# XiandaGuo/OpenStereo

Measured on AMD Instinct MI355X. Metric: stereo-pairs/s at 540x960 D=192 (GwcNet fwd), higher is better.
Workload: dtype f32 via f16x3 split-MFMA (hi/lo fp16 operands, f32 accumulate; HBM tensors f32); 1 GPU; GwcNet-gc inference, SceneFlow-shaped 540x960 padded to 544x960, D=192, G=40 + 12ch concat (BASELINE configs[1]); weights=deterministic synthetic (sharpened), random-init architecture, sub_batch_streams=3, parallelism=independent pairs x1, precision=f16x3, launch=hipGraph replay

## Files before the change

### include/openstereo_amd.h

```cpp
#ifndef OPENSTEREO_AMD_H
#define OPENSTEREO_AMD_H

#include <stddef.h>

#ifdef __cplusplus
extern "C" {
#endif

#define OSA_ABI_VERSION 8
#define OSA_META_FLOATS 128

enum { OSA_NCDHW = 0, OSA_NDHWC = 1 };
enum { OSA_ACT_NONE = 0, OSA_ACT_RELU = 1, OSA_ACT_LEAKY = 2, OSA_ACT_RELU6 = 3, OSA_ACT_SIGMOID = 4, OSA_ACT_TANH = 5 };
enum { OSA_GATE_RAW = 16 };
#define OSA_GATE_CHANNELS(n) ((int)((unsigned)(n) << 16))
enum { OSA_IN_SPLIT = 32, OSA_OUT_SPLIT = 64, OSA_RES_SPLIT = 128, OSA_REDIR_SPLIT = 256 };
enum { OSA_RES_AFTER_ACT = 512 };

int         osa_abi_version(void);
const char* osa_last_error(void);
const char* osa_target_arch(void);

int osa_build_volume_f32(const float* left_gwc, const float* right_gwc, int C, int num_groups,
                         const float* left_cat, const float* right_cat, int Cc,
// ... 310 lines not shown
                     float* out, float* workspace, size_t workspace_bytes, void* stream);
int osa_channel_sums_multi(const void* const* dys, int n_items, int dy_f16, int dy_cs, long long P, int C,
                           float* out, float* workspace, size_t workspace_bytes, void* stream);
int osa_channel_affine(const void* u, int u_f16, int u_cs, const void* v, int v_f16, int v_cs,
                       const float* a, const float* b, const float* c0, void* out, int out_cs,
                       long long P, int C, int relu, void* stream);

size_t osa_instnorm_workspace_floats(int B, long long HW, int C);
int osa_instnorm_nhwc_f32(const float* x, float* y, int B, long long HW, int C, int xCs, int yCs, float eps, int act, float slope,
                          float* workspace, float* y_meta, void* stream);

long long osa_conv3d_march_launches(void);

long long osa_conv3d_march_s2_launches(void);

int osa_conv_b_ring_mask(int mask);
long long osa_conv_b_ring_launches(void);

int osa_volume_walk_step(int step);
long long osa_volume_walk_launches(void);

int osa_build_volume_nhwc_split_eligible(const float* left_cat, const float* right_cat, const float* vol, int C, int num_groups,
                                         int gwc_stride, int Cc, int cat_stride, int vol_channels, int c_off, int W, int maxdisp);
int osa_build_volume_nhwc_split_f16x3(const float* left_gwc, const float* right_gwc, int C, int num_groups, int gwc_stride,
                                      const float* left_cat, const float* right_cat, int Cc, int cat_stride,
                                      float* vol, int vol_channels, int c_off,
                                      int B, int H, int W, int maxdisp, int mask_left_concat,
                                      const float* gwc_meta, const float* cat_meta, float* vol_meta, void* stream);

#ifdef __cplusplus
// ... 4 lines not shown
```

### openstereo_amd/_lib.py

```python
from __future__ import annotations

import ctypes as C
import os
import threading

_HERE = os.path.dirname(os.path.abspath(__file__))
LIB_PATH = os.environ.get("OSA_LIB_PATH") or os.path.join(_HERE, "lib", "libopenstereo_amd.so")

_lock = threading.Lock()
_lib = None

c_fp = C.c_void_p
c_i = C.c_int
c_f = C.c_float
c_st = C.c_void_p
c_ll = C.c_longlong


class F16x3Ranges(C.Structure):
    _fields_ = [("x_meta", C.c_void_p), ("residual_meta", C.c_void_p), ("redir_meta", C.c_void_p),
                ("y_meta", C.c_void_p), ("bound_coef", C.c_void_p), ("redir_bound_coef", C.c_void_p), ("weight_scale", C.c_void_p)]


c_rng = C.POINTER(F16x3Ranges)
# ... 152 lines not shown
                                     c_i, c_f, c_st]),
    "osa_deconv2d_nhwc_f16": (c_i, [c_fp, c_fp, c_fp, c_fp, c_fp, c_fp,
                                    c_i, c_i, c_i, c_i, c_i,
                                    c_i, c_i, c_i,
                                    c_i, c_i, c_i,
                                    c_fp, c_i, c_i, c_f, c_st]),
    "osa_instnorm_workspace_floats": (C.c_size_t, [c_i, c_ll, c_i]),
    "osa_instnorm_nhwc_f32": (c_i, [c_fp, c_fp, c_i, c_ll, c_i, c_i, c_i, c_f, c_i, c_f, c_fp, c_fp, c_st]),
    "osa_conv3d_wgrad_ws_multi": (c_i, [c_i, c_fp, c_fp, c_i, c_fp] + [c_i] * 22 + [c_fp, c_fp, c_i, c_i, c_fp, C.c_size_t, c_st]),
    "osa_channel_sums_workspace_bytes": (C.c_size_t, [c_ll, c_i]),
    "osa_channel_affine": (c_i, [c_fp, c_i, c_i, c_fp, c_i, c_i, c_fp, c_fp, c_fp, c_fp, c_i, c_ll, c_i, c_i, c_st]),
    "osa_channel_sums_multi": (c_i, [c_fp, c_i, c_i, c_i, c_ll, c_i, c_fp, c_fp, C.c_size_t, c_st]),
    "osa_channel_sums": (c_i, [c_fp, c_i, c_i, c_fp, c_i, c_i, c_fp, c_fp, c_fp, c_i, c_ll, c_i, c_fp, c_fp, C.c_size_t, c_st]),
    "osa_conv3d_march_launches": (c_ll, []),
    "osa_conv3d_march_s2_launches": (c_ll, []),
    "osa_conv_b_ring_mask": (c_i, [c_i]),
    "osa_conv_b_ring_launches": (c_ll, []),
    "osa_volume_walk_step": (c_i, [c_i]),
    "osa_volume_walk_launches": (c_ll, []),
    "osa_build_volume_nhwc_split_eligible": (c_i, [c_fp, c_fp, c_fp, c_i, c_i, c_i, c_i, c_i, c_i, c_i, c_i, c_i]),
    "osa_build_volume_nhwc_split_f16x3": (c_i, [c_fp, c_fp, c_i, c_i, c_i, c_fp, c_fp, c_i, c_i, c_fp, c_i, c_i,
                                                c_i, c_i, c_i, c_i, c_i, c_fp, c_fp, c_fp, c_st]),
    "osa_softargmin_f32": (c_i, [c_fp, c_fp, c_i, c_i, c_i, c_i, c_st]),
    "osa_softmax_softargmin_f32": (c_i, [c_fp, c_fp, c_fp, c_i, c_i, c_i, c_i, c_st]),
    "osa_upsample_softargmin_f32": (c_i, [c_fp, c_fp, c_i, c_i, c_i, c_i, c_i, c_i, c_i, c_i, c_st]),
    "osa_softargmin_var_f32": (c_i, [c_fp, c_fp, c_fp, c_fp, c_i, c_i, c_i, c_i, c_st]),
    "osa_softmax_softargmin_var_f32": (c_i, [c_fp, c_fp, c_fp, c_i, c_i, c_i, c_i, c_st]),
    "osa_upsample_softargmin_var_f32": (c_i, [c_fp, c_fp, c_fp, c_i, c_i, c_i, c_i, c_i, c_i, c_i, c_i, c_st]),
    "osa_softargmin_var_bwd_f32": (c_i, [c_fp, c_fp, c_fp, c_fp, c_fp, c_fp, c_i, c_i, c_i, c_i, c_st]),
    "osa_softmax_softargmin_var_bwd_f32": (c_i, [c_fp, c_fp, c_fp, c_fp, c_i, c_i, c_i, c_i, c_st]),
# ... 13 lines not shown
        if _lib is not None:
            return _lib
        if not os.path.exists(LIB_PATH):
            raise EngineError(
                f"{LIB_PATH} is missing: build it with `python -m openstereo_amd.build` "
                "(hipcc, gfx950). There is no CPU fallback.")
        lib = C.CDLL(LIB_PATH)
        for name, (res, args) in SIGNATURES.items():
            fn = getattr(lib, name)
            fn.restype = res
            fn.argtypes = args
        if lib.osa_abi_version() != abi_version(lib):
            raise EngineError(f"ABI version mismatch: library reports {lib.osa_abi_version()}, include/openstereo_amd.h declares {abi_version(lib)}")
        if os.environ.get("OSA_B_RING_MASK"):
            lib.osa_conv_b_ring_mask(int(os.environ["OSA_B_RING_MASK"], 0))
        if os.environ.get("OSA_VOL_WALK"):
            lib.osa_volume_walk_step(int(os.environ["OSA_VOL_WALK"]))
        _lib = lib
    return _lib


_abi = None


def abi_version(lib=None) -> int:
    global _abi
    if _abi is None:
        import re
        hdr = os.path.join(os.path.dirname(os.path.abspath(__file__)), "..", "include", "openstereo_amd.h")
        try:
# ... 22 lines not shown
```

### openstereo_amd/build.py

```python
from __future__ import annotations

import os
import shutil
import subprocess
import sys
from concurrent.futures import ThreadPoolExecutor

HERE = os.path.dirname(os.path.abspath(__file__))
CSRC = os.path.join(HERE, "csrc")
LIBDIR = os.path.join(HERE, "lib")
OBJDIR = os.path.join(LIBDIR, "obj")
LIBNAME = "libopenstereo_amd.so"
SOURCES = ["api.hip", "volume.hip", "conv3d.hip", "conv_inst_f32.hip", "conv_inst_f16x3.hip", "conv_inst_f16.hip", "conv_march.hip", "softargmin.hip", "layout.hip", "refine.hip", "backward.hip", "wgrad.hip", "geometry.hip", "dwconv.hip", "norm.hip", "gru_train.hip"]
ARCH = "gfx950"
HIPCC_FLAGS = ["-O3", "-std=c++17", f"--offload-arch={ARCH}", "-fPIC", "-ffp-contract=off",
               "-Wall", "-Wno-unused-function"]
NO_PACKED_F32 = ["-Xclang", "-target-feature", "-Xclang", "-packed-fp32-ops"]
HIPCC_FLAGS += NO_PACKED_F32
EXTRA_FLAGS: dict = {}


def _hipcc() -> str:
    exe = shutil.which("hipcc") or "/opt/rocm/bin/hipcc"
    if not os.path.exists(exe):
# ... 3 lines not shown

def _stale(target: str, deps: list[str]) -> bool:
    if not os.path.exists(target):
        return True
    t = os.path.getmtime(target)
    return any(os.path.getmtime(d) > t for d in deps)


def lib_path() -> str:
    return os.path.join(LIBDIR, LIBNAME)


def build(force: bool = False, verbose: bool = True) -> str:
    os.makedirs(OBJDIR, exist_ok=True)
    hipcc = _hipcc()
    headers = [os.path.join(CSRC, "osa_common.h"), os.path.join(CSRC, "conv_kernel.h"), os.path.join(CSRC, "conv_march.h"), os.path.join(CSRC, "conv_inst.h"), os.path.join(CSRC, "conv_inst_impl.h"), os.path.join(CSRC, "conv_cfgs.def"),
               os.path.join(HERE, "..", "include", "openstereo_amd.h")]

    def compile_one(src: str) -> str:
        s = os.path.join(CSRC, src)
        o = os.path.join(OBJDIR, src.replace(".hip", ".o"))
        if force or _stale(o, [s, os.path.abspath(__file__)] + headers):
            cmd = [hipcc, *HIPCC_FLAGS, *EXTRA_FLAGS.get(src, []), "-c", s, "-o", o]
            if verbose:
                print("[build]", " ".join(cmd), flush=True)
            subprocess.check_call(cmd)
        return o

    with ThreadPoolExecutor(max_workers=min(len(SOURCES), os.cpu_count() or 1)) as ex:
        objs = list(ex.map(compile_one, SOURCES))
    out = lib_path()
# ... 13 lines not shown
```

### openstereo_amd/csrc/conv3d.hip

```cpp
#include "conv_kernel.h"
#include "conv_inst.h"

namespace osa {

struct KernelCfg {
    const char* name;
    int M, N;
    int TD, TH, TW, threads;
    int ks;
    int table, idx;
};

static const KernelCfg g_cfgs[] = {
#define OSA_CFG_X(RING, MT, NT, WM, WN, TH, TW)                                                                  \
    { #MT "x" #NT "_" #WM "x" #WN "_" #TH "x" #TW, WM * MT * 32, WN * NT * 32, WM * MT * 32 / (TH * TW), TH, TW, WM * WN * 64, 0, 0, -1 },
#define OSA_KS_X(MT, NT, WM, WN, TH, TW, KS)
#include "conv_cfgs.def"
#undef OSA_CFG_X
#undef OSA_KS_X
};
constexpr int N_CFGS = sizeof(g_cfgs) / sizeof(g_cfgs[0]);

static const KernelCfg g_ks_cfgs[] = {
#define OSA_CFG_X(RING, MT, NT, WM, WN, TH, TW)
// ... 148 lines not shown
    const double mfma_per_wave = (double)a.nchunks * a.T * ((double)k.M * k.N / 1024.0 / waves) * (prec == PREC_F16X3 ? 3.0 : 8.0);
    const double tap_us = mfma_per_wave * (prec == PREC_F16X3 ? 32.0 : 64.0) / 2000.0;
    const double bytes = (double)a.LD * a.LH * a.LW * 64.0 * a.nchunks + (double)k.M * (deconv ? 8 : 1) * k.N * 4.0 * (a.res || a.rx ? 2 : 1);
    const double mem_us = bytes / (4.0e6 / 256.0);
    double step_us = tap_us > mem_us ? tap_us : mem_us;
    if ((tap_us + mem_us) / slots > step_us) step_us = (tap_us + mem_us) / slots;
    { const int o = exp_int("OSA_STAG_PCT", 100); step_us *= o / 100.0; }
    { const int o = exp_int("OSA_STAG_US10", 0); if (o) step_us = o / 10.0; }
    a.stag_ticks = (int)(step_us * 100.0 + 0.5);
    a.stag_n = slots * 256; a.stag_cus = 256;
    if (exp_int("OSA_STAG_PRINT", 0)) fprintf(stderr, "[stagger] %s slots %d tap %.2f us mem %.2f us step %.2f us\n", k.name, slots, tap_us, mem_us, step_us);
}

int launch_conv_march(ConvArgs& a, hipStream_t st, const char* what);
int launch_conv_march_s2(ConvArgs& a, hipStream_t st, const char* what);
void wgrad_set_multi_tile(int on);
void march_s2_set_waves(int w);

static int g_b_ring_mask = (1 << 1) | (1 << 2) | (1 << 3) | (1 << 4) | (1 << 13) | (1 << 29) | (1 << 27);
static long long g_b_ring_launches = 0;
static int g_b_ring_mask_value() { return g_b_ring_mask; }

static int launch_conv(ConvArgs& a, int stride, int prec, hipStream_t st, const char* what,
                       const KernelCfg* forced = nullptr) {
#ifdef OSA_EXPERIMENTS
    if (!forced) {
        const int r = launch_conv_pipe(a, stride, prec, st, what);
        if (r != 0) return r < 0 ? r : 0;
    }
#endif
// ... 662 lines not shown
    for (int t = 0; t < d.T; ++t) { a.td[t] = d.dz[t]; a.th[t] = d.dy[t]; a.tw[t] = d.dx[t]; }
    for (int c = 0; c < 8; ++c) a.cls_end[c] = d.cls_end[c];
    a.nchunks = nchunks_of(Ci); a.CoP = pad32(Co);
    a.act = act; a.slope = slope; a.oscale = oscale;
    if (prec == PREC_F16 && f16_units(a, flat ? "deconv2d" : "deconv3d")) return -1;
    if (rx) {
        OSA_REQUIRE(!flat && !residual && !gate_logits, "deconv3d_redir: residual / gate cannot be combined with the fused redir branch");
        OSA_REQUIRE(rw_packed && rCi > 0 && rCi <= 64 && rCi % 4 == 0 && rxCs >= rCi && rxCs % 4 == 0 && ((size_t)rx & 15) == 0,
                    "deconv3d_redir: redir input needs <= 64 channels (multiple of 4), stride >= channels, 16-byte alignment (Ci=%d stride=%d)", rCi, rxCs);
        OSA_REQUIRE((long long)a.Do * a.Ho * a.Wo * rxCs < (1ll << 31), "deconv3d_redir: redir input too large");
        a.rx = rx; a.rxCs = rxCs; a.rCi = rCi; a.rw = reinterpret_cast<const float4*>(rw_packed);
        a.rscale = rscale; a.rshift = rshift; a.roscale = roscale;
    }
    set_ranges(a, rng);
    if (check_split_ranges(a, prec, flat ? "deconv2d" : "deconv3d")) return -1;
    return launch_conv(a, 1, prec, (hipStream_t)stream, flat ? "deconv2d" : "deconv3d",
                       flat ? &g_deconv_flat_cfg : (rx ? (rCi > 32 ? &g_deconv_redir64_cfg : &g_deconv_redir_cfg) : &g_deconv_cfg));
}

#define OSA_DECONV_PARAMS                                                                       \
    const float* x, const float* w_packed, const float* scale, const float* shift,             \
    const float* residual, float* y, int B, int Di, int Hi, int Wi, int Ci, int xCs,           \
    int Co, int yCs, int rCs, int k, int pad, int opad, const float* gate_logits, int gCs, int act, float slope
#define OSA_DECONV_ARGS                                                                         \
    x, w_packed, scale, shift, residual, y, B, Di, Hi, Wi, Ci, xCs, Co, yCs, rCs, k, pad, opad, \
    gate_logits, gCs, act, slope

extern "C" int osa_deconv3d_ndhwc_f32(OSA_DECONV_PARAMS, void* stream) {
    return deconv3d_impl(OSA_DECONV_ARGS, PREC_F32, 1.f, stream);
}
// ... 184 lines not shown
```

### openstereo_amd/csrc/conv_kernel.h

```cpp
#pragma once
#include "osa_common.h"
#include <cstdlib>
#include <cstring>

#include <type_traits>

namespace osa {

typedef float f32x16 __attribute__((ext_vector_type(16)));
typedef _Float16 f16x8 __attribute__((ext_vector_type(8)));
typedef unsigned int u32x4 __attribute__((ext_vector_type(4)));

enum { PREC_F32 = 0, PREC_F16X3 = 1, PREC_F16 = 2 };

constexpr int CC = 16;
constexpr int VS = CC + 4;
constexpr int JO = CC / 8;
constexpr int MAX_TAPS = 64;

struct ConvArgs {
    const float* x; const float4* w; const float* scale; const float* shift; const float* res; float* y;
    const float* gate; int gCs;
    int B, Di, Hi, Wi, Ci, xCs;
    int Do, Ho, Wo, Co, yCs, rCs;
// ... 171 lines not shown
            else if (lane_in) row[lane] = zero;
        } else if (lane_in) row[lane] = zero;
    }
}

__device__ __forceinline__ void wait_vmcnt(const int n) {
    switch (n) {
        case 0: asm volatile("s_waitcnt vmcnt(0)" ::: "memory"); break;
        case 1: asm volatile("s_waitcnt vmcnt(1)" ::: "memory"); break;
        case 2: asm volatile("s_waitcnt vmcnt(2)" ::: "memory"); break;
        case 3: asm volatile("s_waitcnt vmcnt(3)" ::: "memory"); break;
        case 4: asm volatile("s_waitcnt vmcnt(4)" ::: "memory"); break;
        case 5: asm volatile("s_waitcnt vmcnt(5)" ::: "memory"); break;
        default: asm volatile("s_waitcnt vmcnt(6)" ::: "memory"); break;
    }
}

#ifdef OSA_TRACE_ON
constexpr int TRACE_SLOTS = 32, TRACE_WAVES = 4, TRACE_EVENTS = 40;
static __device__ unsigned long long g_trace[TRACE_SLOTS * TRACE_WAVES * TRACE_EVENTS];
#define OSA_TRACE(ev) do { if ((p.dbg & 256) && (tid & 63) == 0 && blockIdx.y == 0 && blockIdx.x % 97 == 0 && blockIdx.x / 97 < TRACE_SLOTS && (tid >> 6) < TRACE_WAVES && (ev) < TRACE_EVENTS) \
    g_trace[((blockIdx.x / 97) * TRACE_WAVES + (tid >> 6)) * TRACE_EVENTS + (ev)] = wall_clock64(); } while (0)
#else
#define OSA_TRACE(ev) do {} while (0)
#endif

template <int PREC, int NCLS, int TU, int MT, int NT, int WM, int WN, int TH, int TW, int REDIR = 0, int OUTS = 0, int PIPE = 0, int KS = 1, int BL = 0>
#ifndef OSA_S2_U
#define OSA_S2_U 12
#endif
// ... 1077 lines not shown
```

### openstereo_amd/csrc/conv_march.h

```cpp
#pragma once
#include "conv_kernel.h"

namespace osa {

template <int NWV, int TW>
struct MarchGeo {
    static constexpr int MT = 2;
    static constexpr int RPT = 32 / TW;
    static constexpr int TH = NWV * MT * RPT;
    static constexpr int LH = TH + 2, LW = TW + 2;
    static constexpr int VQ = 5;
    static constexpr int ROWQ = (TW == 16) ? ((LW * VQ + 15) / 16 * 16) : LW * VQ;
    static constexpr int NPI = (LH * ROWQ + 63) / 64;
    static constexpr int PLANEQ = NPI * 64;
    static constexpr int NP = (NPI + NWV - 1) / NWV;
    static constexpr int NTHR = NWV * 64;
    static constexpr int BRING = 4;
    static constexpr int BSTEPQ = 6 * 64;
    static constexpr size_t lds_bytes() { return (size_t)2 * PLANEQ * 16 + (size_t)BRING * BSTEPQ * 16; }
    static_assert((size_t)NWV * 32 * 36 * 4 <= (size_t)PLANEQ * 16, "epilogue tiles must fit into one plane buffer");
    static_assert(NP <= 7, "one piece per wave and step, all of them forced home by the waits of steps 2..8");
};

__device__ const float4 g_march_zeros[4] = {};

template <int NWV, int TW, int OUTS, int INS>
__global__ __launch_bounds__(NWV * 64, 2) void conv_march_kernel(const ConvArgs p, const int dseg, const int nseg) {
    using G = MarchGeo<NWV, TW>;
    constexpr int MT = G::MT, TH = G::TH, ROWQ = G::ROWQ, VQ = G::VQ, PLANEQ = G::PLANEQ, NTHR = G::NTHR, NP = G::NP, NPI = G::NPI;
    extern __shared__ __attribute__((aligned(16))) float4 smem[];
    float4* const bring = smem + 2 * PLANEQ;

    const int tid = threadIdx.x, lane = tid & 63;
    const int wm = __builtin_amdgcn_readfirstlane(tid >> 6);
    const int col = lane & 31, hh = lane >> 5;

    unsigned bid = xcd_remap(blockIdx.x, gridDim.x);
    const int twi = bid % p.tilesW; bid /= p.tilesW;
    const int thi = bid % p.tilesH; bid /= p.tilesH;
    const int seg = bid % nseg;
// ... 32 lines not shown
            for (int r = 0; r < 16; ++r) acc[s][m][r] = 0.f;

    const int bstep = 2 * p.CoP;
    const int tstep = 2 * bstep;
    const int nch = p.nchunks;

    const int cq = (lane & 7) * 4, vsub = lane >> 3;
    const int c8 = (lane & 3) * 8, vs2 = lane >> 2;
    const int actk = p.act & 15;
    const float act_ns = (actk == OSA_ACT_NONE) ? 1.f : ((actk == OSA_ACT_LEAKY) ? p.slope : 0.f);
    const bool act_relu = actk == OSA_ACT_RELU;
    const size_t ovox_b = (size_t)b * p.Do * p.Ho * p.Wo;
    float* const yb = p.y + ovox_b * p.yCs;
    const float* const resb = p.res ? p.res + ovox_b * p.rCs : nullptr;

    auto dma = [&](const char* src, const unsigned lds_byte) {
        const unsigned m0v = __builtin_amdgcn_readfirstlane(lds_byte);
        unsigned keep;
        asm volatile("s_mov_b32 %0, m0\n\ts_mov_b32 m0, %2\n\ts_nop 0\n\tglobal_load_lds_dwordx4 %1, off\n\ts_mov_b32 m0, %0"
                     : "=&s"(keep) : "v"(src), "s"(m0v) : "memory");
    };
    const unsigned smem_lds = (unsigned)(size_t)(__attribute__((address_space(3))) char*)smem;
    const unsigned bring_lds = smem_lds + 2u * PLANEQ * 16u;
    const char* const zsrc = reinterpret_cast<const char*>(g_march_zeros);

    constexpr int PERW = 384 / NWV, NI = (PERW + 63) / 64;
    unsigned boff[NI];
#pragma unroll
    for (int i = 0; i < NI; ++i) {
        const int j = wm * PERW + i * 64 + lane, f = (j >> 6) < 6 ? (j >> 6) : 5;
        boff[i] = (unsigned)(((f >> 1) * 9 * tstep + (f & 1) * bstep + (j & 63)) * 16);
    }
    auto dma_b = [&](const int slot, const int ch, const int khw) {
        const char* base = reinterpret_cast<const char*>(p.w) + (size_t)(ch * 27 + khw) * tstep * 16;
#pragma unroll
        for (int i = 0; i < NI; ++i)
            if ((i + 1) * 64 <= PERW || i * 64 + lane < PERW)
                dma(base + boff[i], bring_lds + (unsigned)((slot * 384 + wm * PERW + i * 64) * 16));
    };
// ... 202 lines not shown
```

### openstereo_amd/csrc/conv_march.hip

```cpp
#include "conv_march.h"
#include "conv_march_s2.h"

namespace osa {

static long long g_march_launches = 0;
long long march_launches() { return g_march_launches; }

struct MarchCfg { int nwv, tw, th; size_t lds; void (*fn[2][2])(const ConvArgs, int, int); };
#define OSA_MARCH_CFG(NWV, TW) { NWV, TW, MarchGeo<NWV, TW>::TH, MarchGeo<NWV, TW>::lds_bytes(),                      \
                                 { { conv_march_kernel<NWV, TW, 0, 0>, conv_march_kernel<NWV, TW, 0, 1> },            \
                                   { conv_march_kernel<NWV, TW, 1, 0>, conv_march_kernel<NWV, TW, 1, 1> } } }
static const MarchCfg g_march_cfgs[] = {
    OSA_MARCH_CFG(4, 16),
    OSA_MARCH_CFG(4, 32),
};

int launch_conv_march(ConvArgs& a, hipStream_t st, const char* what) {
    if (!exp_int("OSA_MARCH", 1)) return 0;
    if (a.T != 27 || a.Co != 32 || a.CoP != 32 || a.Di < 3 || a.gate || a.rx) return 0;
    if (a.Ci % 16 != 0) return 0;
    const int actk = a.act & 15;
    if (actk > OSA_ACT_LEAKY || (a.act & (OSA_GATE_RAW | OSA_RES_AFTER_ACT)) || ((unsigned)a.act >> 16)) return 0;
    if ((a.yCs & 3) || ((size_t)a.y & 15) || (a.res && ((a.rCs & 3) || ((size_t)a.res & 15)))) return 0;
    if ((long long)a.Do * a.Ho * a.Wo * (a.yCs > a.rCs ? a.yCs : a.rCs) >= (1ll << 31)) return 0;
// ... 91 lines not shown

int launch_conv_march_s2(ConvArgs& a, hipStream_t st, const char* what) {
    if (a.T != 27 || a.Co != 64 || a.CoP != 64 || a.Di < 2 || a.gate || a.rx || a.res) return 0;
    if (a.Ci % 16 != 0 || a.xCs % 16 != 0) return 0;
    if (!(a.act & OSA_IN_SPLIT) || !(a.act & OSA_OUT_SPLIT)) return 0;
    const int actk = a.act & 15;
    if (actk > OSA_ACT_LEAKY || (a.act & (OSA_GATE_RAW | OSA_RES_AFTER_ACT)) || ((unsigned)a.act >> 16)) return 0;
    if ((a.yCs % 16) || ((size_t)a.y & 15) || ((size_t)a.x & 15)) return 0;
    if ((long long)a.Do * a.Ho * a.Wo * a.yCs >= (1ll << 31)) return 0;
    if ((long long)a.Hi * a.Wi * a.xCs >= (1ll << 29)) return 0;
    const int r = g_march_s2_waves == 8 ? launch_conv_march_s2_t<8>(a, st, what) : launch_conv_march_s2_t<4>(a, st, what);
    if (r == 1) ++g_march_s2_launches;
    return r;
}

}

extern "C" long long osa_conv3d_march_launches(void) { return osa::march_launches(); }
extern "C" long long osa_conv3d_march_s2_launches(void) { return osa::march_s2_launches(); }
```

### openstereo_amd/csrc/conv_march_s2.h

```cpp
#pragma once
#include "conv_kernel.h"

namespace osa {

template <int NWV_>
struct MarchS2Geo {
    static constexpr int NWV = NWV_, TW = 32, TH = NWV_ / 2;
    static constexpr int LH = 2 * TH + 1, LW = 2 * TW + 1, NEV = TW + 1;
    static constexpr int NVOX = LH * LW;
    static constexpr int NPI = (NVOX * 4 + 63) / 64;
    static constexpr int PLANEQ = NPI * 64;
    static constexpr int NP = (NPI + NWV - 1) / NWV;
    static constexpr int BRING = 3, BSTEPQ = 12 * 64;
    static constexpr int NIB = NWV == 8 ? 2 : 3;
    static constexpr size_t lds_bytes() { return (size_t)2 * PLANEQ * 16 + (size_t)BRING * BSTEPQ * 16; }
    static_assert((size_t)NWV * 32 * 36 * 4 <= (size_t)PLANEQ * 16, "epilogue tiles must fit into one plane buffer");
};

__device__ const float4 g_march_s2_zeros[4] = {};

template <int N>
__device__ __forceinline__ void wait_vmcnt_c() {
    static_assert(N >= 0 && N <= 15, "vmcnt immediate");
    if constexpr (N == 0) asm volatile("s_waitcnt vmcnt(0)" ::: "memory");
    else if constexpr (N == 1) asm volatile("s_waitcnt vmcnt(1)" ::: "memory");
    else if constexpr (N == 2) asm volatile("s_waitcnt vmcnt(2)" ::: "memory");
    else if constexpr (N == 3) asm volatile("s_waitcnt vmcnt(3)" ::: "memory");
    else if constexpr (N == 4) asm volatile("s_waitcnt vmcnt(4)" ::: "memory");
    else if constexpr (N == 5) asm volatile("s_waitcnt vmcnt(5)" ::: "memory");
    else if constexpr (N == 6) asm volatile("s_waitcnt vmcnt(6)" ::: "memory");
    else if constexpr (N == 7) asm volatile("s_waitcnt vmcnt(7)" ::: "memory");
    else if constexpr (N == 8) asm volatile("s_waitcnt vmcnt(8)" ::: "memory");
    else asm volatile("s_waitcnt vmcnt(9)" ::: "memory");
}
// ... 28 lines not shown
    unsigned amax_seen = 0u;
    if (p.out_meta) amax_seen = amax_peek(p.out_meta);

    f32x16 acc0, acc1;
#pragma unroll
    for (int r = 0; r < 16; ++r) { acc0[r] = 0.f; acc1[r] = 0.f; }

    const int CoP = p.CoP;
    const int nch = p.nchunks;
    const int c8 = (lane & 3) * 8, vs2 = lane >> 2;
    const int actk = p.act & 15;
    const float act_ns = (actk == OSA_ACT_NONE) ? 1.f : ((actk == OSA_ACT_LEAKY) ? p.slope : 0.f);
    const bool act_relu = actk == OSA_ACT_RELU;
    float* const yb = p.y + (size_t)b * p.Do * p.Ho * p.Wo * p.yCs;

    auto dma = [&](const char* src, const unsigned lds_byte) {
        const unsigned m0v = __builtin_amdgcn_readfirstlane(lds_byte);
        unsigned keep;
        asm volatile("s_mov_b32 %0, m0\n\ts_mov_b32 m0, %2\n\ts_nop 0\n\tglobal_load_lds_dwordx4 %1, off\n\ts_mov_b32 m0, %0"
                     : "=&s"(keep) : "v"(src), "s"(m0v) : "memory");
    };
    const unsigned smem_lds = (unsigned)(size_t)(__attribute__((address_space(3))) char*)smem;
    const unsigned bring_lds = smem_lds + 2u * PLANEQ * 16u;
    const char* const zsrc = reinterpret_cast<const char*>(g_march_s2_zeros);

    unsigned boff[NIB], bdst[NIB];
#pragma unroll
    for (int i = 0; i < NIB; ++i) {
        const int f = NWV == 8 ? (i == 0 ? wv : 8 + (wv & 3)) : wv * 3 + i;
        const int kw = f >> 2, hl = (f >> 1) & 1, n = f & 1;
        boff[i] = (unsigned)((kw * 4 * CoP + hl * 2 * CoP + hh * CoP + n * 32 + col) * 16);
        bdst[i] = (unsigned)(f * 64 * 16);
    }
    auto dma_b = [&](const int slot, const int ch, const int kh, const int kd) {
        const char* base = reinterpret_cast<const char*>(p.w) + (size_t)((ch * 27 + kd * 9 + kh * 3) * 4 * CoP) * 16;
#pragma unroll
        for (int i = 0; i < NIB; ++i) dma(base + boff[i], bring_lds + (unsigned)(slot * G::BSTEPQ * 16) + bdst[i]);
    };

// ... 154 lines not shown
```

Measured before the change: 196.6 stereo-pairs/s.

## Add plane-walking transposed-conv3d kernel with fused redir 1x1 epilogue

Measured after the change: 200.2 stereo-pairs/s (median of 6 runs). +1.8%, better.

```diff
diff --git a/include/openstereo_amd.h b/include/openstereo_amd.h
--- a/include/openstereo_amd.h
+++ b/include/openstereo_amd.h
@@ -7,7 +7,7 @@
 extern "C" {
 #endif
 
-#define OSA_ABI_VERSION 8
+#define OSA_ABI_VERSION 9
 #define OSA_META_FLOATS 128
 
 enum { OSA_NCDHW = 0, OSA_NDHWC = 1 };
@@ -348,6 +348,10 @@
 
 long long osa_conv3d_march_s2_launches(void);
 
+int osa_deconv_walk(int enable);
+int osa_deconv_walk_segment_planes(int planes);
+long long osa_deconv3d_walk_launches(void);
+
 int osa_conv_b_ring_mask(int mask);
 long long osa_conv_b_ring_launches(void);
 
diff --git a/openstereo_amd/_lib.py b/openstereo_amd/_lib.py
--- a/openstereo_amd/_lib.py
+++ b/openstereo_amd/_lib.py
@@ -190,6 +190,9 @@
     "osa_channel_sums": (c_i, [c_fp, c_i, c_i, c_fp, c_i, c_i, c_fp, c_fp, c_fp, c_i, c_ll, c_i, c_fp, c_fp, C.c_size_t, c_st]),
     "osa_conv3d_march_launches": (c_ll, []),
     "osa_conv3d_march_s2_launches": (c_ll, []),
+    "osa_deconv_walk": (c_i, [c_i]),
+    "osa_deconv_walk_segment_planes": (c_i, [c_i]),
+    "osa_deconv3d_walk_launches": (c_ll, []),
     "osa_conv_b_ring_mask": (c_i, [c_i]),
     "osa_conv_b_ring_launches": (c_ll, []),
     "osa_volume_walk_step": (c_i, [c_i]),
@@ -233,6 +236,8 @@
             raise EngineError(f"ABI version mismatch: library reports {lib.osa_abi_version()}, include/openstereo_amd.h declares {abi_version(lib)}")
         if os.environ.get("OSA_B_RING_MASK"):
             lib.osa_conv_b_ring_mask(int(os.environ["OSA_B_RING_MASK"], 0))
+        if os.environ.get("OSA_DECONV_WALK"):
+            lib.osa_deconv_walk(int(os.environ["OSA_DECONV_WALK"], 0))
         if os.environ.get("OSA_VOL_WALK"):
             lib.osa_volume_walk_step(int(os.environ["OSA_VOL_WALK"]))
         _lib = lib
diff --git a/openstereo_amd/build.py b/openstereo_amd/build.py
--- a/openstereo_amd/build.py
+++ b/openstereo_amd/build.py
@@ -41,7 +41,7 @@
 def build(force: bool = False, verbose: bool = True) -> str:
     os.makedirs(OBJDIR, exist_ok=True)
     hipcc = _hipcc()
-    headers = [os.path.join(CSRC, "osa_common.h"), os.path.join(CSRC, "conv_kernel.h"), os.path.join(CSRC, "conv_march.h"), os.path.join(CSRC, "conv_inst.h"), os.path.join(CSRC, "conv_inst_impl.h"), os.path.join(CSRC, "conv_cfgs.def"),
+    headers = [os.path.join(CSRC, "osa_common.h"), os.path.join(CSRC, "conv_kernel.h"), os.path.join(CSRC, "conv_march.h"), os.path.join(CSRC, "conv_march_s2.h"), os.path.join(CSRC, "conv_deconv_walk.h"), os.path.join(CSRC, "conv_inst.h"), os.path.join(CSRC, "conv_inst_impl.h"), os.path.join(CSRC, "conv_cfgs.def"),
                os.path.join(HERE, "..", "include", "openstereo_amd.h")]
 
     def compile_one(src: str) -> str:
diff --git a/openstereo_amd/csrc/conv3d.hip b/openstereo_amd/csrc/conv3d.hip
--- a/openstereo_amd/csrc/conv3d.hip
+++ b/openstereo_amd/csrc/conv3d.hip
@@ -186,6 +186,7 @@
 
 int launch_conv_march(ConvArgs& a, hipStream_t st, const char* what);
 int launch_conv_march_s2(ConvArgs& a, hipStream_t st, const char* what);
+int launch_conv_deconv_walk(ConvArgs& a, hipStream_t st, const char* what);
 void wgrad_set_multi_tile(int on);
 void march_s2_set_waves(int w);
 
@@ -878,6 +879,10 @@
     }
     set_ranges(a, rng);
     if (check_split_ranges(a, prec, flat ? "deconv2d" : "deconv3d")) return -1;
+    if (prec == PREC_F16X3 && !flat && k == 3 && rx) {
+        const int r = launch_conv_deconv_walk(a, (hipStream_t)stream, "deconv3d (walk)");
+        if (r != 0) return r < 0 ? r : 0;
+    }
     return launch_conv(a, 1, prec, (hipStream_t)stream, flat ? "deconv2d" : "deconv3d",
                        flat ? &g_deconv_flat_cfg : (rx ? (rCi > 32 ? &g_deconv_redir64_cfg : &g_deconv_redir_cfg) : &g_deconv_cfg));
 }
diff --git a/openstereo_amd/csrc/conv_deconv_walk.h b/openstereo_amd/csrc/conv_deconv_walk.h
--- /dev/null
+++ b/openstereo_amd/csrc/conv_deconv_walk.h
@@ -0,0 +1,287 @@
+#pragma once
+#include "conv_march_s2.h"
+
+namespace osa {
+
+template <int WN_>
+struct DeconvWalkGeo {
+    static constexpr int NWV = 4, WN = WN_, WM = NWV / WN_, MT = 2, TW = 32, TH = WM * MT;
+    static constexpr int LH = TH + 1, LW = TW + 1, VQ = 5, ROWQ = LW * VQ;
+    static constexpr int NPI = (LH * ROWQ + 63) / 64;
+    static constexpr int TILEQ = NWV * 32 * 36 / 4;
+    static constexpr int PLANEQ = (NPI * 64 > TILEQ) ? NPI * 64 : TILEQ;
+    static constexpr int NP = (NPI + NWV - 1) / NWV;
+    static constexpr int BRING = 3, NFRAG = 6 * WN_, BSTEPQ = NFRAG * 64;
+    static constexpr int NIB = (NFRAG + NWV - 1) / NWV;
+    static constexpr size_t lds_bytes() { return (size_t)2 * PLANEQ * 16 + (size_t)BRING * BSTEPQ * 16; }
+    static_assert(NIB + NP <= 9, "vmcnt immediates of the step waits");
+};
+
+template <int WN_, int RCH>
+__global__ __launch_bounds__(256, 2) void conv_deconv_walk_kernel(const ConvArgs p, const int oseg, const int nseg) {
+    using G = DeconvWalkGeo<WN_>;
+    constexpr int PLANEQ = G::PLANEQ, NP = G::NP, NPI = G::NPI, NWV = G::NWV, NIB = G::NIB, WN = G::WN, MT = G::MT, TH = G::TH, TW = G::TW,
+                  ROWQ = G::ROWQ, VQ = G::VQ;
+    extern __shared__ __attribute__((aligned(16))) float4 smem[];
+    float4* const bring = smem + 2 * PLANEQ;
+
+    const int tid = threadIdx.x, lane = tid & 63;
+    const int wv = __builtin_amdgcn_readfirstlane(tid >> 6);
+    const int wm = wv / WN, wn = wv % WN;
+    const int col = lane & 31, hh = lane >> 5;
+
+    unsigned bid = xcd_remap(blockIdx.x, gridDim.x);
+    const int twi = bid % p.tilesW; bid /= p.tilesW;
+    const int thi = bid % p.tilesH; bid /= p.tilesH;
+    const int seg = bid % nseg;
+    const int b = (int)(bid / nseg);
+    const int o0 = seg * oseg, o1 = (o0 + oseg < p.Do) ? o0 + oseg : p.Do;
+    const int a0h = thi * TH, a0w = twi * TW;
+
+    float s_in = 1.f, s_rx = 1.f, s_out = 1.f;
+    if (p.in_meta) s_in = p.in_meta[1];
+    if (p.rx_meta) s_rx = p.rx_meta[1];
+    if (p.coef && p.in_meta) {
+        float bound = p.coef[0] * amax_read(p.in_meta) + p.coef[1];
+        if (p.rcoef && p.rx_meta) bound += p.rcoef[0] * amax_read(p.rx_meta) + p.rcoef[1];
+        s_out = pow2_scale(bound * 1.0625f);
+    }
+    if (p.out_meta && blockIdx.x == 0 && tid == 0) p.out_meta[1] = s_out;
+    const float osc = (p.wscale_dev ? p.wscale_dev[1] : p.oscale) * (1.0f / s_in);
+    const float rosc = p.roscale * (1.0f / s_rx);
+    float am = 0.f;
+    unsigned amax_seen = 0u;
+    if (p.out_meta) amax_seen = amax_peek(p.out_meta);
+
+    f32x16 acc[4][MT];
+    auto zero_acc = [&]() {
+#pragma unroll
+        for (int c = 0; c < 4; ++c)
+#pragma unroll
+            for (int m = 0; m < MT; ++m)
+#pragma unroll
+                for (int r = 0; r < 16; ++r) acc[c][m][r] = 0.f;
+    };
+    zero_acc();
+
+    const int CoP = p.CoP;
+    const int nch = p.nchunks;
+    const int c8 = (lane & 3) * 8, vs2 = lane >> 2;
+    const int actk = p.act & 15;
+    const float act_ns = (actk == OSA_ACT_NONE) ? 1.f : ((actk == OSA_ACT_LEAKY) ? p.slope : 0.f);
+    const bool act_relu = actk == OSA_ACT_RELU;
+    const size_t ovox_b = (size_t)b * p.Do * p.Ho * p.Wo;
+    float* const yb = p.y + ovox_b * p.yCs;
+    const float* const rxb = p.rx + ovox_b * p.rxCs;
+
+    const int cl = wn * 32 + col;
+    const float s6 = p.scale ? p.scale[cl] * osc : osc, t6 = p.shift ? p.shift[cl] : 0.f;
+    const float sr = p.rscale ? p.rscale[cl] * rosc : rosc, tr = p.rshift ? p.rshift[cl] : 0.f;
+    const float4* const rwp = p.rw + (size_t)hh * CoP + cl;
+    const int rbstep = 2 * CoP, rtstep = JO * rbstep;
+    constexpr bool HOIST_W = (RCH == 2);
+    float4 rwb[HOIST_W ? RCH : 1][2];
+    if constexpr (HOIST_W) {
+#pragma unroll
+        for (int ch = 0; ch < RCH; ++ch) { rwb[ch][0] = rwp[ch * rtstep]; rwb[ch][1] = rwp[ch * rtstep + rbstep]; }
+    }
+
+    auto dma = [&](const char* src, const unsigned lds_byte) { lds_dma16(src, lds_byte); };
+    const unsigned smem_lds = (unsigned)(size_t)(__attribute__((address_space(3))) char*)smem;
+    const unsigned bring_lds = smem_lds + 2u * PLANEQ * 16u;
+    const char* const zsrc = reinterpret_cast<const char*>(g_lds_dma_zeros);
+
+    int bkw[NIB];
+    unsigned boff[NIB], bdst[NIB];
+#pragma unroll
+    for (int i = 0; i < NIB; ++i) {
+        const int f = (WN == 1) ? (i == 0 ? wv : 4 + (wv & 1)) : wv * 3 + i;
+        const int hl = (f / WN) & 1, n = f % WN;
+        bkw[i] = f / (2 * WN);
+        boff[i] = (unsigned)(((hl * 2 + hh) * CoP + n * 32 + col) * 16);
+        bdst[i] = (unsigned)(f * 64 * 16);
+    }
+    auto dma_b = [&](const int slot, const int ch, const int kd, const int kh) {
+        const char* base = reinterpret_cast<const char*>(p.w) + (size_t)(ch * 27) * (4 * CoP * 16);
+#pragma unroll
+        for (int i = 0; i < NIB; ++i) {
+            const int t = p.toff[kd * 9 + kh * 3 + bkw[i]];
+            dma(base + (size_t)t * (4 * CoP * 16) + boff[i], bring_lds + (unsigned)(slot * G::BSTEPQ * 16) + bdst[i]);
+        }
+    };
+
+    unsigned poff[NP];
+    unsigned pvalid = 0u;
+#pragma unroll
+    for (int i = 0; i < NP; ++i) {
+        int n = i * NWV + wv;
+        n = n < NPI ? n : NPI - 1;
+        const int j = n * 64 + lane;
+        const int lh = j / ROWQ, rem = j - lh * ROWQ, lw = rem / VQ, c4 = rem - lw * VQ;
+        const int gh = a0h + lh, gw = a0w + lw;
+        const bool ok = lh < G::LH && c4 < 4 && gh < p.Hi && gw < p.Wi;
+        poff[i] = ok ? (unsigned)(((gh * p.Wi + gw) * p.xCs + c4 * 4) * 4) : 0u;
+        pvalid |= ok ? (1u << i) : 0u;
+    }
+    const size_t plane_bytes = (size_t)p.Hi * p.Wi * p.xCs * 4;
+    const char* const xb = reinterpret_cast<const char*>(p.x) + (size_t)b * p.Di * plane_bytes;
+    auto dma_plane = [&](const int buf, const int pd, const int c) {
+        const char* base = xb + (size_t)(pd < 0 ? 0 : pd) * plane_bytes + (size_t)c * (CC * 4);
+#pragma unroll
+        for (int i = 0; i < NP; ++i) {
+            int n = i * NWV + wv;
+            n = n < NPI ? n : NPI - 1;
+            const bool ok = ((pvalid >> i) & 1u) && pd >= 0;
+            dma(ok ? base + poff[i] : zsrc, smem_lds + (unsigned)((buf * PLANEQ + n * 64) * 16));
+        }
+    };
+
+    auto taps = [&](auto KH_, const int cur, const int slot) {
+        constexpr int KH = decltype(KH_)::value;
+        constexpr int ph = (KH != 1) ? 1 : 0, dh = (KH == 0) ? 1 : 0;
+#pragma unroll
+        for (int kw = 0; kw < 3; ++kw) {
+            const int pw = (kw != 1) ? 1 : 0, dw = (kw == 0) ? 1 : 0;
+            float4 A[MT][2], Bf[2];
+#pragma unroll
+            for (int m = 0; m < MT; ++m) {
+                const int v = cur * PLANEQ + (wm * MT + m + dh) * ROWQ + (col + dw) * VQ + hh;
+                A[m][0] = smem[v]; A[m][1] = smem[v + 2];
+            }
+            Bf[0] = bring[slot * G::BSTEPQ + ((kw * 2 + 0) * WN + wn) * 64 + lane];
+            Bf[1] = bring[slot * G::BSTEPQ + ((kw * 2 + 1) * WN + wn) * 64 + lane];
+#pragma unroll
+            for (int term = 0; term < 3; ++term)
+#pragma unroll
+                for (int m = 0; m < MT; ++m) {
+                    const f16x8 a = __builtin_bit_cast(f16x8, A[m][term == 1 ? 1 : 0]);
+                    const f16x8 w = __builtin_bit_cast(f16x8, Bf[term == 0 ? 1 : 0]);
+                    acc[ph * 2 + pw][m] = __builtin_amdgcn_mfma_f32_32x32x16_f16(a, w, acc[ph * 2 + pw][m], 0, 0, 0);
+                }
+        }
+    };
+
+    auto epilogue = [&](const int od, float* const tb) {
+        constexpr int RV = 2 * RCH;
+        auto load_x = [&](const int i, float4 (&rv)[RV]) {
+            const int c = i / MT, m = i % MT;
+            const int ih = a0h + wm * MT + m, iw = a0w + col;
+            const bool ok = ih < p.Hi && iw < p.Wi;
+            const int vox = (od * p.Ho + 2 * ih + (c >> 1)) * p.Wo + 2 * iw + (c & 1);
+#pragma unroll
+            for (int k = 0; k < RV; ++k) {
+                rv[k] = make_float4(0.f, 0.f, 0.f, 0.f);
+                if (ok) rv[k] = *reinterpret_cast<const float4*>(rxb + vox * p.rxCs + (k >> 1) * CC + 4 * hh + 8 * (k & 1));
+            }
+        };
+        float4 rv[RV];
+        load_x(0, rv);
+#pragma unroll
+        for (int i = 0; i < 4 * MT; ++i) {
+            const int c = i / MT, m = i % MT;
+            f32x16 r;
+#pragma unroll
+            for (int e = 0; e < 16; ++e) r[e] = 0.f;
+#pragma unroll
+            for (int ch = 0; ch < RCH; ++ch) {
+                float4 b0, b1;
+                if constexpr (HOIST_W) { b0 = rwb[ch][0]; b1 = rwb[ch][1]; }
+                else { b0 = rwp[ch * rtstep]; b1 = rwp[ch * rtstep + rbstep]; }
+                const f16x8 ah = __builtin_bit_cast(f16x8, rv[2 * ch]), al = __builtin_bit_cast(f16x8, rv[2 * ch + 1]);
+                const f16x8 bh = __builtin_bit_cast(f16x8, b0), bl = __builtin_bit_cast(f16x8, b1);
+                r = __builtin_amdgcn_mfma_f32_32x32x16_f16(ah, bl, r, 0, 0, 0);
+                r = __builtin_amdgcn_mfma_f32_32x32x16_f16(al, bh, r, 0, 0, 0);
+                r = __builtin_amdgcn_mfma_f32_32x32x16_f16(ah, bh, r, 0, 0, 0);
+            }
+            __builtin_amdgcn_sched_barrier(0);
+            if (i + 1 < 4 * MT) load_x(i + 1, rv);
+#pragma unroll
+            for (int e = 0; e < 16; ++e) tb[((e & 3) + 8 * (e >> 2) + 4 * hh) * 36 + col] = fmaf(acc[c][m][e], s6, t6) + fmaf(r[e], sr, tr);
+            const int ih = a0h + wm * MT + m;
+            const int soff = wn * 32 + (c8 >> 4) * 16 + ((c8 & 15) >> 3) * 4;
+#pragma unroll
+            for (int k = 0; k < 2; ++k) {
+                const int iw = a0w + vs2 + 16 * k;
+                const bool ok = ih < p.Hi && iw < p.Wi;
+                const int vox = (od * p.Ho + 2 * ih + (c >> 1)) * p.Wo + 2 * iw + (c & 1);
+                uint2 hq[2], lq[2];
+#pragma unroll
+                for (int h2 = 0; h2 < 2; ++h2) {
+                    const float4 a = *reinterpret_cast<const float4*>(tb + (vs2 + 16 * k) * 36 + c8 + 4 * h2);
+                    float o[4] = {a.x, a.y, a.z, a.w};
+#pragma unroll
+                    for (int e = 0; e < 4; ++e) o[e] = (o[e] < 0.f) ? (act_relu ? 0.f : o[e] * act_ns) : o[e];
+                    if (ok) am = fmaxf(am, fmaxf(fmaxf(fabsf(o[0]), fabsf(o[1])), fmaxf(fabsf(o[2]), fabsf(o[3]))));
+                    split_f16(make_float4(o[0] * s_out, o[1] * s_out, o[2] * s_out, o[3] * s_out), hq[h2], lq[h2]);
+                }
+                if (ok) {
+                    float* ys = yb + vox * p.yCs + soff;
+                    store16(ys, make_uint4(hq[0].x, hq[0].y, hq[1].x, hq[1].y));
+                    store16(ys + 8, make_uint4(lq[0].x, lq[0].y, lq[1].x, lq[1].y));
+                }
+            }
+            __builtin_amdgcn_sched_barrier(0);
+        }
+    };
+
+    auto nsrc = [&](const int od) { return (od & 1) ? (((od >> 1) + 1 < p.Di) ? 2 : 1) : 1; };
+    auto kd_of = [&](const int od, const int j) { return (od & 1) ? (j == 0 ? 2 : 0) : 1; };
+    int lod = o0, lj = 0, lc = 0, lk = 0;
+    bool ldone = false;
+    auto issue_b = [&](const int slot) {
+        dma_b(slot, lc, kd_of(lod, lj), lk);
+        if (!ldone) {
+            if (++lk == 3) {
+                lk = 0;
+                if (++lc == nch) { lc = 0; if (++lj == nsrc(lod)) { lj = 0; ++lod; } }
+                if (lod >= o1) { ldone = true; lod = o1 - 1; lj = nsrc(lod) - 1; lc = nch - 1; lk = 2; }
+            }
+        }
+    };
+
+    dma_plane(0, o0 >> 1, 0);
+    issue_b(0); issue_b(1);
+    wait_vmcnt_c<0>();
+
+    int slot = 0;
+    int q = 0;
+    for (int od = o0; od < o1; ++od) {
+        const int ns = nsrc(od);
+        int cur = 0;
+        for (int j = 0; j < ns; ++j)
+            for (int c = 0; c < nch; ++c, ++q) {
+                cur = q & 1;
+                int nod = od, nj = j, nc = c + 1;
+                if (nc == nch) { nc = 0; if (++nj == ns) { nj = 0; ++nod; } }
+                const int npd = (nod < o1) ? (nod >> 1) + nj : -1;
+                __syncthreads();
+                issue_b(slot >= 1 ? slot - 1 : 2);
+                dma_plane(cur ^ 1, npd, nc);
+                taps(std::integral_constant<int, 0>{}, cur, slot);
+                wait_vmcnt_c<NIB + NP>();
+                slot = slot == 2 ? 0 : slot + 1;
+
+                __syncthreads();
+                issue_b(slot >= 1 ? slot - 1 : 2);
+                taps(std::integral_constant<int, 1>{}, cur, slot);
+                wait_vmcnt_c<NIB + NP>();
+                slot = slot == 2 ? 0 : slot + 1;
+
+                __syncthreads();
+                issue_b(slot >= 1 ? slot - 1 : 2);
+                taps(std::integral_constant<int, 2>{}, cur, slot);
+                wait_vmcnt_c<NIB>();
+                slot = slot == 2 ? 0 : slot + 1;
+            }
+        __syncthreads();
+        epilogue(od, reinterpret_cast<float*>(smem + cur * PLANEQ) + wv * (32 * 36));
+        zero_acc();
+    }
+    wait_vmcnt_c<0>();
+    if (p.out_meta) {
+        __syncthreads();
+        publish_amax(p.out_meta, am, amax_seen, reinterpret_cast<float*>(smem));
+    }
+}
+
+}
diff --git a/openstereo_amd/csrc/conv_kernel.h b/openstereo_amd/csrc/conv_kernel.h
--- a/openstereo_amd/csrc/conv_kernel.h
+++ b/openstereo_amd/csrc/conv_kernel.h
@@ -209,6 +209,14 @@
         case 5: asm volatile("s_waitcnt vmcnt(5)" ::: "memory"); break;
         default: asm volatile("s_waitcnt vmcnt(6)" ::: "memory"); break;
     }
+}
+
+__device__ const float4 g_lds_dma_zeros[4] = {};
+__device__ __forceinline__ void lds_dma16(const char* src, const unsigned lds_byte) {
+    const unsigned m0v = __builtin_amdgcn_readfirstlane(lds_byte);
+    unsigned keep;
+    asm volatile("s_mov_b32 %0, m0\n\ts_mov_b32 m0, %2\n\ts_nop 0\n\tglobal_load_lds_dwordx4 %1, off\n\ts_mov_b32 m0, %0"
+                 : "=&s"(keep) : "v"(src), "s"(m0v) : "memory");
 }
 
 #ifdef OSA_TRACE_ON
diff --git a/openstereo_amd/csrc/conv_march.h b/openstereo_amd/csrc/conv_march.h
--- a/openstereo_amd/csrc/conv_march.h
+++ b/openstereo_amd/csrc/conv_march.h
@@ -22,8 +22,6 @@
     static_assert(NP <= 7, "one piece per wave and step, all of them forced home by the waits of steps 2..8");
 };
 
-__device__ const float4 g_march_zeros[4] = {};
-
 template <int NWV, int TW, int OUTS, int INS>
 __global__ __launch_bounds__(NWV * 64, 2) void conv_march_kernel(const ConvArgs p, const int dseg, const int nseg) {
     using G = MarchGeo<NWV, TW>;
@@ -86,15 +84,10 @@
     float* const yb = p.y + ovox_b * p.yCs;
     const float* const resb = p.res ? p.res + ovox_b * p.rCs : nullptr;
 
-    auto dma = [&](const char* src, const unsigned lds_byte) {
-        const unsigned m0v = __builtin_amdgcn_readfirstlane(lds_byte);
-        unsigned keep;
-        asm volatile("s_mov_b32 %0, m0\n\ts_mov_b32 m0, %2\n\ts_nop 0\n\tglobal_load_lds_dwordx4 %1, off\n\ts_mov_b32 m0, %0"
-                     : "=&s"(keep) : "v"(src), "s"(m0v) : "memory");
-    };
+    auto dma = [&](const char* src, const unsigned lds_byte) { lds_dma16(src, lds_byte); };
     const unsigned smem_lds = (unsigned)(size_t)(__attribute__((address_space(3))) char*)smem;
     const unsigned bring_lds = smem_lds + 2u * PLANEQ * 16u;
-    const char* const zsrc = reinterpret_cast<const char*>(g_march_zeros);
+    const char* const zsrc = reinterpret_cast<const char*>(g_lds_dma_zeros);
 
     constexpr int PERW = 384 / NWV, NI = (PERW + 63) / 64;
     unsigned boff[NI];
diff --git a/openstereo_amd/csrc/conv_march.hip b/openstereo_amd/csrc/conv_march.hip
--- a/openstereo_amd/csrc/conv_march.hip
+++ b/openstereo_amd/csrc/conv_march.hip
@@ -1,5 +1,6 @@
 #include "conv_march.h"
 #include "conv_march_s2.h"
+#include "conv_deconv_walk.h"
 
 namespace osa {
 
@@ -129,7 +130,69 @@
     return r;
 }
 
+static long long g_deconv_walk_launches = 0;
+long long deconv_walk_launches() { return g_deconv_walk_launches; }
+
+static int g_deconv_walk = 2;
+int deconv_walk_set(int enable) { const int prev = g_deconv_walk; g_deconv_walk = enable & 3; return prev; }
+static int g_deconv_walk_planes = 0;
+int deconv_walk_planes_set(int planes) { const int prev = g_deconv_walk_planes; g_deconv_walk_planes = planes > 0 ? planes : 0; return prev; }
+
+template <int WN, int RCH>
+static int launch_conv_deconv_walk_t(ConvArgs& a, hipStream_t st, const char* what) {
+    using G = DeconvWalkGeo<WN>;
+    a.tilesD = 1; a.tilesH = cdiv(a.Hi, G::TH); a.tilesW = cdiv(a.Wi, G::TW);
+    for (int t = 0, c = 0; t < a.T; ++t) {
+        while (t >= a.cls_end[c]) ++c;
+        const int kd = ((c >> 2) & 1) ? (a.td[t] == 1 ? 0 : 2) : 1;
+        const int kh = ((c >> 1) & 1) ? (a.th[t] == 1 ? 0 : 2) : 1;
+        const int kw = (c & 1) ? (a.tw[t] == 1 ? 0 : 2) : 1;
+        a.toff[kd * 9 + kh * 3 + kw] = t;
+    }
+    const long long cols = (long long)a.B * a.tilesH * a.tilesW;
+    const long long slots = 2 * 256;
+    int nseg = 1;
+    {
+        double best = 1e30;
+        for (int n = 1; n <= a.Do; ++n) {
+            const int os = cdiv(a.Do, n), ns = cdiv(a.Do, os);
+            if (ns != n) continue;
+            const double cost = (double)((cols * ns + slots - 1) / slots) * (1.5 * os + 0.5);
+            if (cost < best - 1e-9) { best = cost; nseg = ns; }
+        }
+    }
+    int oseg = cdiv(a.Do, nseg);
+    if (g_deconv_walk_planes > 0) oseg = g_deconv_walk_planes < a.Do ? g_deconv_walk_planes : a.Do;
+    nseg = cdiv(a.Do, oseg);
+    OSA_REQUIRE(cols * nseg < (1ll << 31), "%s: grid too large", what);
+    OSA_REQUIRE(hipFuncSetAttribute((const void*)conv_deconv_walk_kernel<WN, RCH>, hipFuncAttributeMaxDynamicSharedMemorySize, (int)G::lds_bytes()) == hipSuccess,
+                "%s: %d bytes of LDS per workgroup refused", what, (int)G::lds_bytes());
+    hipLaunchKernelGGL((conv_deconv_walk_kernel<WN, RCH>), dim3((unsigned)(cols * nseg)), dim3(G::NWV * 64), G::lds_bytes(), st, a, oseg, nseg);
+    OSA_LAUNCH_CHECK(what);
+    return 1;
+}
+
+int launch_conv_deconv_walk(ConvArgs& a, hipStream_t st, const char* what) {
+    if (a.T != 27 || a.Do != 2 * a.Di || a.Ho != 2 * a.Hi || a.Wo != 2 * a.Wi) return 0;
+    if (!a.rx || a.res || a.gate) return 0;
+    const int cls = (a.Co == 32 && a.rCi == 32) ? 0 : ((a.Co == 64 && a.rCi == 64) ? 1 : -1);
+    if (cls < 0 || a.CoP != a.Co || !((g_deconv_walk >> cls) & 1)) return 0;
+    if (!(a.act & OSA_IN_SPLIT) || !(a.act & OSA_OUT_SPLIT) || !(a.act & OSA_REDIR_SPLIT)) return 0;
+    const int actk = a.act & 15;
+    if (actk > OSA_ACT_LEAKY || (a.act & (OSA_GATE_RAW | OSA_RES_AFTER_ACT)) || ((unsigned)a.act >> 16)) return 0;
+    if (a.Ci % 16 != 0 || a.xCs % 16 != 0 || a.yCs % 16 != 0 || a.rxCs % 16 != 0) return 0;
+    if (((size_t)a.x & 15) || ((size_t)a.y & 15) || ((size_t)a.rx & 15)) return 0;
+    if ((long long)a.Do * a.Ho * a.Wo * (a.yCs > a.rxCs ? a.yCs : a.rxCs) >= (1ll << 31)) return 0;
+    if ((long long)a.Hi * a.Wi * a.xCs >= (1ll << 29)) return 0;
+    const int r = cls == 0 ? launch_conv_deconv_walk_t<1, 2>(a, st, what) : launch_conv_deconv_walk_t<2, 4>(a, st, what);
+    if (r == 1) ++g_deconv_walk_launches;
+    return r;
+}
+
 }
 
 extern "C" long long osa_conv3d_march_launches(void) { return osa::march_launches(); }
 extern "C" long long osa_conv3d_march_s2_launches(void) { return osa::march_s2_launches(); }
+extern "C" long long osa_deconv3d_walk_launches(void) { return osa::deconv_walk_launches(); }
+extern "C" int osa_deconv_walk(int enable) { return osa::deconv_walk_set(enable); }
+extern "C" int osa_deconv_walk_segment_planes(int planes) { return osa::deconv_walk_planes_set(planes); }
diff --git a/openstereo_amd/csrc/conv_march_s2.h b/openstereo_amd/csrc/conv_march_s2.h
--- a/openstereo_amd/csrc/conv_march_s2.h
+++ b/openstereo_amd/csrc/conv_march_s2.h
@@ -16,8 +16,6 @@
     static constexpr size_t lds_bytes() { return (size_t)2 * PLANEQ * 16 + (size_t)BRING * BSTEPQ * 16; }
     static_assert((size_t)NWV * 32 * 36 * 4 <= (size_t)PLANEQ * 16, "epilogue tiles must fit into one plane buffer");
 };
-
-__device__ const float4 g_march_s2_zeros[4] = {};
 
 template <int N>
 __device__ __forceinline__ void wait_vmcnt_c() {
@@ -76,15 +74,10 @@
     const bool act_relu = actk == OSA_ACT_RELU;
     float* const yb = p.y + (size_t)b * p.Do * p.Ho * p.Wo * p.yCs;
 
-    auto dma = [&](const char* src, const unsigned lds_byte) {
-        const unsigned m0v = __builtin_amdgcn_readfirstlane(lds_byte);
-        unsigned keep;
-        asm volatile("s_mov_b32 %0, m0\n\ts_mov_b32 m0, %2\n\ts_nop 0\n\tglobal_load_lds_dwordx4 %1, off\n\ts_mov_b32 m0, %0"
-                     : "=&s"(keep) : "v"(src), "s"(m0v) : "memory");
-    };
+    auto dma = [&](const char* src, const unsigned lds_byte) { lds_dma16(src, lds_byte); };
     const unsigned smem_lds = (unsigned)(size_t)(__attribute__((address_space(3))) char*)smem;
     const unsigned bring_lds = smem_lds + 2u * PLANEQ * 16u;
-    const char* const zsrc = reinterpret_cast<const char*>(g_march_s2_zeros);
+    const char* const zsrc = reinterpret_cast<const char*>(g_lds_dma_zeros);
 
     unsigned boff[NIB], bdst[NIB];
 #pragma unroll
```
